# kharchenkolab/dropEst

Hardware: AMD Instinct MI355X
Metric: Mreads/s processed to final count matrix (higher is better)
Workload: dtype u64

## Files before the change

dropest_amd/capi.py:

```python
import ctypes as C
import os

import numpy as np

from .build import LIB, build

ESCAPE = 1 << 63
NO_GENE = 0xFFFFFFFF

MERGE_NONE, MERGE_REAL_BARCODES, MERGE_SIMPLE, MERGE_POISSON_REAL, MERGE_POISSON_SIMPLE, MERGE_ALL = 0, 1, 2, 3, 4, 5
BARCODES_INDROP, BARCODES_CONST = 0, 1
UMI_MERGE_SIMPLE, UMI_MERGE_DIRECTIONAL = 0, 1

_STATUS = {1: "INVALID", 2: "RANGE", 3: "DEVICE", 4: "UNSUPPORTED", 5: "IO"}


class MatrixBytes(C.Structure):
    _fields_ = [("ncols", C.c_uint64), ("nnz", C.c_uint64), ("colptr", C.c_void_p), ("row_delta", C.c_void_p), ("value", C.c_void_p),
                ("n_row_listed", C.c_uint64), ("row_listed_pos", C.c_void_p), ("row_listed_row", C.c_void_p),
                ("n_value_listed", C.c_uint64), ("value_listed_pos", C.c_void_p), ("value_listed_value", C.c_void_p)]


class DropestError(RuntimeError):
    def __init__(self, status, msg):
# ... 158 lines not shown
        "dropest_sort_layout": (C.c_int, [vp, C.POINTER(C.c_uint32)]),
        "dropest_stream": (vp, [vp]),
        "dropest_host_register": (C.c_int, [C.c_int, vp, C.c_uint64, P(vp)]),
        "dropest_host_unregister": (C.c_int, [C.c_int, vp]),
        "dropest_ingest": (C.c_int, [vp]),
        "dropest_ingest_summary_get": (C.c_int, [vp, P(IngestSummary)]),
        "dropest_ingest_summary_set": (C.c_int, [vp, P(IngestSummary)]),
        "dropest_gene_chr_table": (C.c_int, [vp, P(vp), u64p]),
        "dropest_shard_merge_search": (C.c_int, [vp, C.c_uint64, vp, vp, vp, C.c_uint64, vp, vp, u64p]),
        "dropest_shard_merge_pairs": (C.c_int, [vp, vp, vp]),
        "dropest_shard_merge_export": (C.c_int, [vp, u64p, vp, vp, P(vp), vp]),
        "dropest_shard_merge_intersect": (C.c_int, [vp, C.c_uint64, vp, vp, vp, vp, vp]),
        "dropest_shard_merge_decide": (C.c_int, [vp, vp, vp]),
        "dropest_merge_apply": (C.c_int, [C.c_uint64, C.c_uint64, vp, vp, vp, vp, vp, vp]),
        "dropest_shard_merge_finish": (C.c_int, [vp, C.c_uint64, vp, vp, vp, vp, vp, C.c_uint64, vp, vp, C.c_uint64, vp, vp, vp]),
        "dropest_synth_generate_host": (C.c_int, [P(SynthParams), C.c_uint64, C.c_uint64, vp, vp, vp, vp]),
        "dropest_synth_generate_device": (C.c_int, [P(SynthParams), C.c_int, C.c_uint64, C.c_uint64, vp, vp, vp, vp]),
        "dropest_dev_alloc": (C.c_int, [C.c_int, C.c_uint64, P(vp)]),
        "dropest_dev_free": (C.c_int, [C.c_int, vp]),
        "dropest_dev_copy_to_host": (C.c_int, [C.c_int, vp, vp, C.c_uint64]),
        "dropest_dev_copy_from_host": (C.c_int, [C.c_int, vp, vp, C.c_uint64]),
        "dropest_dev_count": (C.c_int, []),
        "dropest_dev_sync": (C.c_int, [C.c_int]),
        "dropest_rand_sequence": (C.c_int, [C.c_uint32, C.c_uint64, vp]),
        "dropest_table_sizes": (C.c_int, [vp, vp]),
        "dropest_shard_unique_id": (C.c_int, [vp]),
        "dropest_shard_create": (C.c_int, [P(Cfg), C.c_int32, C.c_int32, vp, P(vp)]),
        "dropest_shard_group_create": (C.c_int, [P(Cfg), C.c_int32, vp, vp]),
        "dropest_shard_destroy": (None, [vp]),
        "dropest_shard_ctx": (vp, [vp]),
        "dropest_shard_set_reads_device": (C.c_int, [vp, vp, vp, vp, vp, C.c_uint64, C.c_uint64]),
        "dropest_shard_step": (C.c_int, [vp]),
        "dropest_shard_push_reads": (C.c_int, [vp, vp, vp, vp, vp, C.c_uint64, C.c_uint64]),
        "dropest_shard_push_reads_device": (C.c_int, [vp, vp, vp, vp, vp, C.c_uint64, C.c_uint64, C.c_int32, vp]),
        "dropest_deal_range": (C.c_int, [C.c_uint64, C.c_uint64, C.c_uint64, C.c_int32, vp, P(C.c_uint32)]),
        "dropest_reserve_reads": (C.c_int, [vp, C.c_uint64]),
        "dropest_shard_group_step": (C.c_int, [vp, C.c_int32]),
        "dropest_shard_merge_validation_samples": (C.c_int, [vp, P(ValidationOpts), P(ValidationSample), C.c_uint32]),
        "dropest_shard_group_merge_validation_samples": (C.c_int, [vp, C.c_int32, P(ValidationOpts), P(ValidationSample), C.c_uint32]),
        "dropest_validation_cut_pairs": (C.c_int, [vp, C.c_uint64, C.c_int32, vp]),
        "dropest_shard_read_corrections": (C.c_int, [vp, u64p, u64p, P(vp), P(vp), P(vp)]),
        "dropest_shard_group_read_corrections": (C.c_int, [vp, C.c_int32]),
        "dropest_shard_group_read_corrections_host": (C.c_int, [vp, C.c_int32, C.c_uint64, C.c_uint64, vp, vp, vp]),
        "dropest_shard_group_read_correction_counts": (C.c_int, [vp, C.c_int32, vp]),
        "dropest_shard_filtered_barcodes_device": (C.c_int, [vp, u64p, P(vp)]),
        "dropest_shard_matrix": (C.c_int, [vp, C.c_int, u64p, u64p, P(vp), P(vp), P(vp), P(vp)]),
# ... 15 lines not shown
    return L


EXPORTED_SYMBOLS = [
    "dropest_last_error", "dropest_cfg_defaults", "dropest_ctx_create", "dropest_ctx_destroy",
    "dropest_set_side_strings", "dropest_push_reads", "dropest_push_reads_device", "dropest_set_initialized",
    "dropest_merge_and_filter", "dropest_reset_results", "dropest_total_cells", "dropest_real_cells",
    "dropest_cell_rows", "dropest_cell_id_by_cb", "dropest_filtered_cells", "dropest_merge_targets",
    "dropest_global_counters", "dropest_cell_molecules", "dropest_molecules", "dropest_count_matrix",
    "dropest_count_matrix_csc", "dropest_count_matrix_csc_levels", "dropest_owner_of", "dropest_partition_by_owner", "dropest_partition_scratch_bytes", "dropest_clear_reads",
    "dropest_count_matrix_device", "dropest_cell_first_reads_device", "dropest_assemble_columns", "dropest_assemble_columns_async",
    "dropest_real_candidate_rows", "dropest_dev_copy_device", "dropest_umi_distribution",
    "dropest_collisions_adjusted_sizes", "dropest_poisson_intersection_prob", "dropest_poisson_upper_tail",
    "dropest_merge_validation", "dropest_merge_validation_samples",
    "dropest_shard_merge_validation_samples", "dropest_shard_group_merge_validation_samples", "dropest_validation_cut_pairs",
    "dropest_set_umi_qualities", "dropest_umi_quality_length", "dropest_cell_molecule_qualities",
    "dropest_set_umi_qualities_var", "dropest_cell_molecule_quality_lengths",
    "dropest_exclude_cell", "dropest_merge_cells", "dropest_merge_umis",
    "dropest_chr_stats", "dropest_merge_target", "dropest_simple_merge_pairs", "dropest_kernel_stats", "dropest_set_profiling", "dropest_set_profiling_filter", "dropest_prefetch_raw_matrix", "dropest_radix_plan", "dropest_stream",
    "dropest_sort_layout", "dropest_host_register", "dropest_host_unregister", "dropest_ingest", "dropest_ingest_summary_get", "dropest_ingest_summary_set",
    "dropest_gene_chr_table", "dropest_shard_merge_search", "dropest_shard_merge_pairs", "dropest_shard_merge_export",
    "dropest_shard_merge_intersect", "dropest_shard_merge_decide", "dropest_merge_apply", "dropest_shard_merge_finish",
    "dropest_synth_generate_host", "dropest_synth_generate_device", "dropest_dev_alloc", "dropest_dev_free",
    "dropest_dev_copy_to_host", "dropest_dev_copy_from_host", "dropest_dev_count", "dropest_dev_sync",
    "dropest_rand_sequence", "dropest_table_sizes",
    "dropest_shard_unique_id", "dropest_shard_create", "dropest_shard_group_create", "dropest_shard_destroy", "dropest_shard_ctx",
    "dropest_shard_set_reads_device", "dropest_shard_push_reads", "dropest_shard_push_reads_device", "dropest_deal_range", "dropest_reserve_reads", "dropest_shard_step", "dropest_shard_group_step", "dropest_shard_matrix", "dropest_shard_matrix_form",
    "dropest_shard_merged_barcodes", "dropest_shard_phase_stats", "dropest_shard_set_option", "dropest_test_transport", "dropest_plan_columns",
    "dropest_key_width", "dropest_ctx_split", "dropest_shard_matrix_narrow", "dropest_shard_matrix_bytes", "dropest_add_umi_to_cell", "dropest_umi_first_seen", "dropest_resident_reads", "dropest_prefetch_raw_matrix_narrow", "dropest_narrow_matrix_possible", "dropest_count_matrix_csc_narrow",
    "dropest_prefetch_raw_matrix_bytes", "dropest_count_matrix_csc_bytes", "dropest_matrix_bytes_widen", "dropest_matrix_rider_widen", "dropest_set_raw_matrix_prefetch", "dropest_set_matrix_wire", "dropest_set_umi_dictionary", "dropest_debug_refresh", "dropest_push_reads_gather", "dropest_shard_set_umi_qualities", "dropest_shard_set_umi_qualities_var",
    "dropest_debug_poison_scratch", "dropest_debug_trim_pool", "dropest_debug_alloc_ordinal", "dropest_debug_alloc_site",
    "dropest_set_save_umi_merge_targets", "dropest_umi_merge_targets", "dropest_read_corrections", "dropest_read_corrections_host",
    "dropest_read_correction_counts", "dropest_cell_barcodes_device",
    "dropest_shard_read_corrections", "dropest_shard_group_read_corrections", "dropest_shard_group_read_corrections_host",
    "dropest_shard_group_read_correction_counts", "dropest_shard_filtered_barcodes_device",
]


_B2C = {"A": 0, "C": 1, "G": 2, "T": 3}


def pack_seq(s):
    if not s or len(s) > 31:
        return None
    c = 1
    for ch in s:
        b = _B2C.get(ch)
# ... 656 lines not shown
```

dropest_amd/csrc/dropest_amd.hip:

```cpp

#include "context.h"
extern "C" void dropest_bgzf_warm_up(void *stream);
#include "k_keyscatter.h"
#include "k_umidict.h"

#include <atomic>
#include <functional>
#include <map>
#include <mutex>

using namespace dropest;

static thread_local std::string g_last_error;

template <class F>
static dropest_status guarded(F &&f) {
	try {
		f();
		return DROPEST_OK;
	} catch (const InvalidError &e) { g_last_error = e.what(); return DROPEST_ERR_INVALID;
	} catch (const RangeError &e) { g_last_error = e.what(); return DROPEST_ERR_RANGE;
	} catch (const UnsupportedError &e) { g_last_error = e.what(); return DROPEST_ERR_UNSUPPORTED;
	} catch (const IoError &e) { g_last_error = e.what(); return DROPEST_ERR_IO;
	} catch (const DeviceError &e) { g_last_error = e.what(); return DROPEST_ERR_DEVICE;
// ... 878 lines not shown
	const u32 rounds = 256;
	std::vector<u32> h(size_t(rounds) * 64), got(size_t(rounds) * 64);
	u32 x = 2463534242u;
	for (u32 r = 0; r < rounds; ++r) {
		const u32 nd = 1u + r % 64u;
		for (u32 l = 0; l < 64; ++l) { x ^= x << 13; x ^= x >> 17; x ^= x << 5; h[size_t(r) * 64 + l] = (x >> 8) % nd; }
	}
	DevBuf<u32> d_in, d_out;
	d_in.alloc(h.size()); d_out.alloc(h.size());
	HIP_CHECK(hipMemcpyAsync(d_in.p, h.data(), h.size() * 4, hipMemcpyHostToDevice, stream));
	hipLaunchKernelGGL(ss_lds_order_probe_kernel, dim3(1), dim3(64), 0, stream, d_in.p, rounds, d_out.p);
	HIP_CHECK(hipGetLastError());
	HIP_CHECK(hipMemcpyAsync(got.data(), d_out.p, got.size() * 4, hipMemcpyDeviceToHost, stream));
	HIP_CHECK(stream_wait(stream));
	bool ordered = true;
	for (u32 r = 0; r < rounds && ordered; ++r) {
		u32 seen[64] = {0};
		for (u32 l = 0; l < 64; ++l) { const u32 d = h[size_t(r) * 64 + l]; if (got[size_t(r) * 64 + l] != seen[d]) ordered = false; ++seen[d]; }
	}
	if (!ordered) fprintf(stderr, "[dropest_amd] device %d: LDS atomics of one instruction are not applied in lane order here; the finishing sort of the splitter sort ranks with ballots (slower, same results)\n", device);
	return known[device] = ordered;
}

bool dropest_ctx::splitter_sort_reduce() {
	const u32 n = u32(n_reads);
	const SsPlan plan = ss_plan(n_reads, chr_from_gene, layout.val_bytes);
	if (!plan.applicable) return false;
	const int tb = plan.tb, fb1 = plan.fb1, fb2 = plan.fb2;
	const bool wide = fb2 > 9;
	const u32 F1 = 1u << fb1, Ff = 1u << fb2, F2 = F1 * Ff;
	const int ms = layout.mark_shift, VB = layout.val_bytes;
	(void)tb;
	uint64_t os_max = plan.os;
	if (const char *e = getenv("DROPEST_SSORT_OS")) os_max = uint64_t(std::max(1, atoi(e)));
	const u32 os = u32(std::max<uint64_t>(1, std::min<uint64_t>(os_max, uint64_t(n) / (uint64_t(F2) * 2))));
	const u32 n_sample = F2 * os;
	const u64 order_mask = ~((1ull << ms) - 1ull);
	const u64 varying = (counters.key_or ^ counters.key_and) & order_mask;
	const bool reserve = plan.reserve && !ss_no_reserve && keys_a.n >= plan.span && keys_b.n >= plan.span &&
	                     (!VB || (vals_a.bytes() >= plan.span && vals_b.bytes() >= plan.span));
	const size_t span = reserve ? size_t(plan.span) : size_t(n);

	HostStage hs(this, "splitter_sort");
	u64 *keys = keys_a.p, *keys_alt = keys_b.p;
	uint8_t *vals = reinterpret_cast<uint8_t *>(vals_a.p), *vals_alt = reinterpret_cast<uint8_t *>(vals_b.p);

	const bool in_l1 = keys_in_l1 && reserve;
	if (keys_in_l1 && !reserve) throw InvalidError("internal: keys partitioned by the key pass, but the sort does not place by reservation");
	const bool rebase = VB == 1 && ms == 0 && reserve && !in_l1 && !getenv("DROPEST_SS_NO_REBASE");
	const int VB2 = rebase ? 0 : VB, ms2 = rebase ? 3 : ms;
	const u64 rebase_mask = rebase ? ~((1ull << layout.umi_bits) - 1ull) : 0ull;
	if (!in_l1) {
		ss_sample_a.ensure(n_sample); ss_sample_b.ensure(n_sample); ss_fine.ensure(F2); ss_coarse.ensure(F1);
		timed("ss_sample", double(n_sample) * 16, [&] {
			hipLaunchKernelGGL(ss_sample_kernel, dim3(div_up(n_sample, 256)), dim3(256), 0, stream, keys, n, ms, n_sample, ss_sample_a.p);
		});
		ss_splitters_from_sample(n_sample, os, Ff, F2, varying >> ms);
	}

	const u32 n_tiles = div_up(n, SS_TILE);
	u32 nblocks = std::min<u32>(n_tiles, 1024);
	const u32 tpb = div_up(n_tiles, nblocks);
	nblocks = div_up(n_tiles, tpb);
	const u32 parts = std::max<u32>(1, std::min<u32>(16, 2048 / F1));
	ss_bucket_base.ensure(F2); ss_bucket_cnt.ensure(F2); scalars.ensure(16);
	HIP_CHECK(hipMemsetAsync(scalars.p, 0, 16, stream));
	u32 max_cnt = 0;
	static const u32 SMALL_MAX = [] { const char *e = getenv("DROPEST_SS_SMALL_MAX"); return e && atoi(e) >= 256 && atoi(e) <= 2048 ? u32(atoi(e)) : 2048u; }();
	const bool atomic_rank = lds_atomics_lane_ordered(cfg.device, stream);
	ss_tmp.ensure(span * 2 + 2); ss_n_loc.ensure(F2); ss_prefix.ensure(F2); ss_chunk.ensure(1024);
	SsLocalArgs a{};
	a.keys = keys; a.vals = vals; a.bucket_base = ss_bucket_base.p; a.bucket_cnt = ss_bucket_cnt.p; a.n_buckets = F2; a.ms = ms2;
	if (rebase) { a.rebase_coarse = ss_coarse.p; a.rebase_mask = rebase_mask; a.rebase_div = Ff; }
	a.t_key = keys_alt; a.t_reads = ss_tmp.p; a.t_agg = ss_tmp.p + span; a.n_loc = ss_n_loc.p;
	if (const char *e = getenv("DROPEST_SS_DEBUG")) a.debug = u32(atoi(e));
	a.order_flag = scalars.p + 2;
	a.atomic_below = u32(ms2 + layout.umi_bits);
	if (const char *e = getenv("DROPEST_SS_ATOMIC_BELOW")) a.atomic_below = u32(atoi(e));
	a.cap = SMALL_MAX; a.skip_above = SMALL_MAX;
	const bool fused_cg_off = getenv("DROPEST_SS_NO_FUSED_CG") != nullptr;
	const bool fuse_cg = !fused_cg_off;
	cg_from_sort = false;
	if (fuse_cg) {
		ss_cg_loc.ensure(F2); ss_cg_cnt.ensure(F2); ss_cg_prefix.ensure(F2);
		HIP_CHECK(hipMemsetAsync(ss_cg_loc.p, 0, size_t(F2) * 4, stream));
		a.cg_loc = ss_cg_loc.p; a.cg_shift = ms2 + layout.umi_bits;
	}
	auto launch_small = [&] {
		static const int wave_mode = [] { const char *e = getenv("DROPEST_SS_LOCAL_WAVE"); return e ? atoi(e) : 0; }();
		if ((wave_mode == 64 || wave_mode == 128) && atomic_rank) {
			const size_t lds1 = ss_local_lds_bytes(a.cap, wave_mode);
			timed(VB2 ? "ss_local:key+1B" : "ss_local:keys", double(n) * (8 + VB2), [&] {
				if (wave_mode == 64) { if (VB2) hipLaunchKernelGGL((ss_local_wave_kernel<64, 1, true>), dim3(F2), dim3(64), lds1, stream, a); else hipLaunchKernelGGL((ss_local_wave_kernel<64, 0, true>), dim3(F2), dim3(64), lds1, stream, a); }
				else { if (VB2) hipLaunchKernelGGL((ss_local_wave_kernel<128, 1, true>), dim3(F2), dim3(128), lds1, stream, a); else hipLaunchKernelGGL((ss_local_wave_kernel<128, 0, true>), dim3(F2), dim3(128), lds1, stream, a); }
			});
			return;
		}
		const size_t lds = ss_local_lds_bytes(a.cap, 256);
		timed(VB2 ? "ss_local:key+1B" : "ss_local:keys", double(n) * (8 + VB2), [&] {
			if (atomic_rank) { if (VB2) hipLaunchKernelGGL((ss_local_kernel<1, true>), dim3(F2), dim3(256), lds, stream, a); else hipLaunchKernelGGL((ss_local_kernel<0, true>), dim3(F2), dim3(256), lds, stream, a); }
			else if (VB2) hipLaunchKernelGGL(ss_local_kernel<1>, dim3(F2), dim3(256), lds, stream, a);
			else hipLaunchKernelGGL(ss_local_kernel<0>, dim3(F2), dim3(256), lds, stream, a);
		});
	};
	if (reserve) {
		const u32 cap1 = u32(plan.cap1), cap2 = u32(plan.cap2), CS1 = 32;
		ss_cursors.ensure(size_t(F1) * CS1 + F2);
		if (!in_l1) HIP_CHECK(hipMemsetAsync(ss_cursors.p, 0, (size_t(F1) * CS1 + F2) * 4, stream));
		else HIP_CHECK(hipMemcpyAsync(scalars.p + 3, ks_flag.p, 4, hipMemcpyDeviceToDevice, stream));
		u32 *cur1 = ss_cursors.p, *cur2 = ss_cursors.p + size_t(F1) * CS1;
		const u32 probe = [] { const char *e = getenv("DROPEST_SS_PROBE"); return e ? u32(atoi(e)) : 0u; }();
		const bool no256 = getenv("DROPEST_SS_NO_F256") != nullptr;
		const u32 rebase_bits = [] { const char *e = getenv("DROPEST_SS_REBASE_BITS"); return e ? u32(std::min(61, std::max(1, atoi(e)))) : 61u; }();
		const SsReserve r1{cur1, CS1, cap1, 0u, scalars.p + 3, probe, rebase_bits}, r2{cur2, 1u, cap2, 0u, scalars.p + 3, probe, 61u};
		if (!in_l1) timed(VB ? "ss_scatter:L1:key+1B" : "ss_scatter:L1:keys", double(n) * (8 + VB + 8 + VB2), [&] {
			auto go = [&](auto kernel) { hipLaunchKernelGGL(kernel, dim3(nblocks), dim3(SS_T), 0, stream, keys, vals, keys_alt, vals_alt, n, ms, fb1, ss_coarse.p, tpb, r1, rebase_mask); };
			if (rebase) { if (wide) go(ss_scatter_res_l1_kernel<1, 1024, true>); else if (fb1 <= 8 && !no256) go(ss_scatter_res_l1_kernel<1, 256, true>); else go(ss_scatter_res_l1_kernel<1, 512, true>); }
			else if (wide) { if (VB) go(ss_scatter_res_l1_kernel<1, 1024>); else go(ss_scatter_res_l1_kernel<0, 1024>); }
			else if (fb1 <= 8 && !no256) { if (VB) go(ss_scatter_res_l1_kernel<1, 256>); else go(ss_scatter_res_l1_kernel<0, 256>); }
			else { if (VB) go(ss_scatter_res_l1_kernel<1, 512>); else go(ss_scatter_res_l1_kernel<0, 512>); }
		});
		timed(VB2 ? "ss_scatter:L2:key+1B" : "ss_scatter:L2:keys", double(n) * 2 * (8 + VB2), [&] {
			auto go = [&](auto kernel) { hipLaunchKernelGGL(kernel, dim3(F1 * parts), dim3(SS_T), 0, stream, keys_alt, vals_alt, keys, vals, ms2, fb2, ss_fine.p, cur1, CS1, cap1, parts, r2,
			                                                 rebase ? ss_coarse.p : static_cast<const u64 *>(nullptr), rebase_mask); };
			if (wide) { if (VB2) go(ss_scatter_res_l2_kernel<1, 1024>); else go(ss_scatter_res_l2_kernel<0, 1024>); }
			else if (fb2 <= 8 && !no256) { if (VB2) go(ss_scatter_res_l2_kernel<1, 256>); else go(ss_scatter_res_l2_kernel<0, 256>); }
			else { if (VB2) go(ss_scatter_res_l2_kernel<1, 512>); else go(ss_scatter_res_l2_kernel<0, 512>); }
		});
		timed("ss_scan", double(F2) * 12, [&] {
			hipLaunchKernelGGL(ss_res_buckets_kernel, dim3(div_up(F2, 256)), dim3(256), 0, stream, cur2, F2, cap2, ss_bucket_base.p, ss_bucket_cnt.p, scalars.p);
		});
		launch_small();
		u32 head[4] = {0, 0, 0, 0};
		fetch(head, scalars.p, 16);
		max_cnt = head[0];
		if (head[3]) {
			stats["count:ss_reserve_overflow"].launches += 1;
			ss_no_reserve = true;
			build_keys(false);
			return splitter_sort_reduce();
		}
		if (max_cnt > SS_LOCAL_MAX) { build_keys(false, false); return false; }
	} else {
	rs_hist.ensure(size_t(F1) * nblocks); rs_row_total.ensure(1024); ss_base1.ensure(F1 + 1);
	timed("ss_hist:L1", double(n) * 8, [&] {
		if (wide) hipLaunchKernelGGL(ss_hist_l1_kernel<1024>, dim3(nblocks), dim3(SS_T), 0, stream, keys, n, ms, fb1, ss_coarse.p, tpb, rs_hist.p);
		else hipLaunchKernelGGL(ss_hist_l1_kernel<512>, dim3(nblocks), dim3(SS_T), 0, stream, keys, n, ms, fb1, ss_coarse.p, tpb, rs_hist.p);
	});
	timed("ss_scan", double(F1) * nblocks * 8, [&] {
		hipLaunchKernelGGL(rs_scan_rows_kernel, dim3(F1), dim3(256), 0, stream, rs_hist.p, nblocks, rs_row_total.p);
		if (wide) hipLaunchKernelGGL(ss_scan_totals_kernel<1024>, dim3(1), dim3(1024), 0, stream, rs_row_total.p, F1, n, ss_base1.p);
		else hipLaunchKernelGGL(ss_scan_totals_kernel<512>, dim3(1), dim3(512), 0, stream, rs_row_total.p, F1, n, ss_base1.p);
	});
	timed(VB ? "ss_scatter:L1:key+1B" : "ss_scatter:L1:keys", double(n) * 2 * (8 + VB), [&] {
		auto go = [&](auto kernel) { hipLaunchKernelGGL(kernel, dim3(nblocks), dim3(SS_T), 0, stream, keys, vals, keys_alt, vals_alt, n, ms, fb1, ss_coarse.p, tpb, rs_hist.p, ss_base1.p); };
		if (wide) { if (VB) go(ss_scatter_l1_kernel<1, 1024>); else go(ss_scatter_l1_kernel<0, 1024>); }
		else { if (VB) go(ss_scatter_l1_kernel<1, 512>); else go(ss_scatter_l1_kernel<0, 512>); }
	});

	ss_cnt2.ensure(size_t(F2) * parts);
	timed("ss_hist:L2", double(n) * 8, [&] {
		if (wide) hipLaunchKernelGGL(ss_hist_l2_kernel<1024>, dim3(F1 * parts), dim3(SS_T), 0, stream, keys_alt, ms, fb2, ss_fine.p, ss_base1.p, parts, ss_cnt2.p);
		else hipLaunchKernelGGL(ss_hist_l2_kernel<512>, dim3(F1 * parts), dim3(SS_T), 0, stream, keys_alt, ms, fb2, ss_fine.p, ss_base1.p, parts, ss_cnt2.p);
	});
	timed("ss_scan", double(F2) * parts * 8, [&] {
		if (wide) hipLaunchKernelGGL(ss_scan_seg_kernel<1024>, dim3(F1), dim3(1024), 0, stream, ss_cnt2.p, Ff, parts, ss_base1.p, ss_bucket_base.p, ss_bucket_cnt.p, scalars.p);
		else hipLaunchKernelGGL(ss_scan_seg_kernel<512>, dim3(F1), dim3(512), 0, stream, ss_cnt2.p, Ff, parts, ss_base1.p, ss_bucket_base.p, ss_bucket_cnt.p, scalars.p);
	});
	fetch(&max_cnt, scalars.p, 4);
	if (max_cnt > SS_LOCAL_MAX) return false;
	timed(VB ? "ss_scatter:L2:key+1B" : "ss_scatter:L2:keys", double(n) * 2 * (8 + VB), [&] {
		auto go = [&](auto kernel) { hipLaunchKernelGGL(kernel, dim3(F1 * parts), dim3(SS_T), 0, stream, keys_alt, vals_alt, keys, vals, ms, fb2, ss_fine.p, ss_base1.p, parts, ss_cnt2.p); };
		if (wide) { if (VB) go(ss_scatter_l2_kernel<1, 1024>); else go(ss_scatter_l2_kernel<0, 1024>); }
		else { if (VB) go(ss_scatter_l2_kernel<1, 512>); else go(ss_scatter_l2_kernel<0, 512>); }
	});
	}

	if (!reserve) launch_small();
	if (max_cnt > SMALL_MAX) {
		std::vector<u32> cnts(F2), medium, big;
		fetch(cnts.data(), ss_bucket_cnt.p, size_t(F2) * 4);
		for (u32 b = 0; b < F2; ++b) if (cnts[b] > SMALL_MAX) (cnts[b] <= 4096 ? medium : big).push_back(b);
		ss_big_list.ensure(medium.size() + big.size());
		if (!medium.empty()) HIP_CHECK(hipMemcpyAsync(ss_big_list.p, medium.data(), medium.size() * 4, hipMemcpyHostToDevice, stream));
		if (!big.empty()) HIP_CHECK(hipMemcpyAsync(ss_big_list.p + medium.size(), big.data(), big.size() * 4, hipMemcpyHostToDevice, stream));
		auto launch = [&](auto kernel, u32 threads, u32 cap, const u32 *list, size_t count) {
			SsLocalArgs g = a;
			g.big_list = list; g.cap = cap; g.skip_above = cap;
			const size_t lds = ss_local_lds_bytes(cap, int(threads));
			HIP_CHECK(hipFuncSetAttribute(reinterpret_cast<const void *>(kernel), hipFuncAttributeMaxDynamicSharedMemorySize, int(lds)));
			hipLaunchKernelGGL(kernel, dim3(u32(count)), dim3(threads), lds, stream, g);
		};
		timed("ss_local:big", 0, [&] {
			if (atomic_rank) {
				if (!medium.empty()) { if (VB2) launch(ss_local_big_kernel<256, 1, true>, 256, 4096, ss_big_list.p, medium.size()); else launch(ss_local_big_kernel<256, 0, true>, 256, 4096, ss_big_list.p, medium.size()); }
				if (!big.empty()) { if (VB2) launch(ss_local_big_kernel<512, 1, true>, 512, SS_LOCAL_MAX, ss_big_list.p + medium.size(), big.size()); else launch(ss_local_big_kernel<512, 0, true>, 512, SS_LOCAL_MAX, ss_big_list.p + medium.size(), big.size()); }
			} else {
				if (!medium.empty()) { if (VB2) launch(ss_local_big_kernel<256, 1>, 256, 4096, ss_big_list.p, medium.size()); else launch(ss_local_big_kernel<256, 0>, 256, 4096, ss_big_list.p, medium.size()); }
				if (!big.empty()) { if (VB2) launch(ss_local_big_kernel<512, 1>, 512, SS_LOCAL_MAX, ss_big_list.p + medium.size(), big.size()); else launch(ss_local_big_kernel<512, 0>, 512, SS_LOCAL_MAX, ss_big_list.p + medium.size(), big.size()); }
			}
		});
		HIP_CHECK(stream_wait(stream));
	}
	const u32 n_chunks = div_up(F2, 1024);
	timed("ss_scan", double(F2) * 12, [&] {
		hipLaunchKernelGGL(ss_chunk_sums_kernel<1024>, dim3(n_chunks), dim3(1024), 0, stream, ss_n_loc.p, F2, ss_chunk.p);
		hipLaunchKernelGGL(ss_prefix_kernel<1024>, dim3(n_chunks), dim3(1024), 0, stream, ss_n_loc.p, F2, ss_chunk.p, n_chunks, ss_prefix.p, scalars.p + 1);
		if (fuse_cg) {
			hipLaunchKernelGGL(ss_cg_counts_kernel, dim3(div_up(F2, 256)), dim3(256), 0, stream, ss_bucket_base.p, ss_n_loc.p, keys_alt, layout.umi_bits, F2, ss_cg_loc.p, ss_cg_cnt.p);
			hipLaunchKernelGGL(ss_chunk_sums_kernel<1024>, dim3(n_chunks), dim3(1024), 0, stream, ss_cg_cnt.p, F2, ss_chunk.p);
			hipLaunchKernelGGL(ss_prefix_kernel<1024>, dim3(n_chunks), dim3(1024), 0, stream, ss_cg_cnt.p, F2, ss_chunk.p, n_chunks, ss_cg_prefix.p, scalars.p + 4);
		}
// ... 1780 lines not shown
```

dropest_amd/csrc/k_ssort.h:

```cpp
#pragma once

#include "util.h"

namespace dropest {

constexpr int SS_T = 512, SS_I = 8, SS_TILE = SS_T * SS_I;
constexpr int SS_MAX_F = 512;
constexpr uint32_t SS_LOCAL_MAX = 8192;

__global__ __launch_bounds__(256) void ss_sample_kernel(const unsigned long long *__restrict__ keys, uint32_t n, int ms,
                                                        uint32_t n_sample, unsigned long long *__restrict__ out) {
	const uint32_t j = blockIdx.x * 256 + threadIdx.x;
	if (j >= n_sample) return;
	const uint32_t pos = uint32_t((uint64_t(j) * n + n / 2) / n_sample);
	out[j] = keys[pos < n ? pos : n - 1] >> ms;
}

__global__ __launch_bounds__(256) void ss_pick_splitters_kernel(const unsigned long long *__restrict__ sorted_sample, uint32_t os, uint32_t F, uint32_t F2,
                                                                unsigned long long *__restrict__ fine, unsigned long long *__restrict__ coarse) {
	const uint32_t j = blockIdx.x * 256 + threadIdx.x;
	if (j >= F2) return;
	const unsigned long long v = j + 1 < F2 ? sorted_sample[size_t(j + 1) * os] : ~0ull;
	fine[j] = v;
	if ((j + 1) % F == 0) coarse[(j + 1) / F - 1] = v;
// ... 294 lines not shown
			if (g < (rs.first + d + 1u) * rs.cap) {
				if constexpr (REBASE) {
					const unsigned long long diff = sk[q] - (d ? (sp[d - 1u] & rebase_mask) : 0ull);
					if (diff >> rs.rebase_bits) atomicOr(rs.overflow, 1u);
					okeys[g] = (diff << 3) | (unsigned long long)(sv[q] & 7u);
				} else {
					okeys[g] = sk[q];
					if (VB) ovals[g] = sv[q];
				}
			}
		}
		if ((rs.dbg & 2u) && t0 + SS_TILE < end) load_tile(t0 + SS_TILE);
		lds_barrier();
	}
}

#define SS_SCATTER_RES_LDS(VB, MAXF)                                                                        \
	__shared__ unsigned long long sp[MAXF];                                                                 \
	__shared__ uint32_t cnt[MAXF], tstart[MAXF], gdelta[MAXF], scratch[SS_T / 64 + 1];                      \
	__shared__ unsigned long long sk[SS_TILE];                                                              \
	__shared__ uint16_t sd[SS_TILE];                                                                        \
	__shared__ uint8_t sv[VB ? SS_TILE : 1];

template <int VB, int MAXF, bool REBASE = false>
__global__ __launch_bounds__(SS_T) void ss_scatter_res_l1_kernel(const unsigned long long *__restrict__ keys, const uint8_t *__restrict__ vals,
                                                                 unsigned long long *__restrict__ okeys, uint8_t *__restrict__ ovals, uint32_t n,
                                                                 int ms, int fb, const unsigned long long *__restrict__ coarse,
                                                                 uint32_t tiles_per_block, SsReserve rs, unsigned long long rebase_mask) {
	SS_SCATTER_RES_LDS(VB, MAXF)
	const uint32_t F = 1u << fb;
	for (uint32_t j = threadIdx.x; j < F; j += SS_T) sp[j] = j + 1 < F ? coarse[j] : ~0ull;
	__syncthreads();
	const uint64_t b64 = uint64_t(blockIdx.x) * tiles_per_block * SS_TILE;
	uint64_t e64 = b64 + uint64_t(tiles_per_block) * SS_TILE;
	if (e64 > n) e64 = n;
	if (b64 < n) ss_scatter_res_range<VB, MAXF, REBASE>(keys, vals, okeys, ovals, uint32_t(b64), uint32_t(e64), ms, fb, sp, rs, cnt, tstart, gdelta, scratch, sk, sd, sv, rebase_mask);
}
template <int VB, int MAXF>
__global__ __launch_bounds__(SS_T) void ss_scatter_res_l2_kernel(const unsigned long long *__restrict__ keys, const uint8_t *__restrict__ vals,
                                                                 unsigned long long *__restrict__ okeys, uint8_t *__restrict__ ovals, int ms, int fb,
                                                                 const unsigned long long *__restrict__ fine, const uint32_t *__restrict__ cur1,
                                                                 uint32_t cstride1, uint32_t cap1, uint32_t parts, SsReserve rs,
                                                                 const unsigned long long *__restrict__ rebase_coarse, unsigned long long rebase_mask) {
	SS_SCATTER_RES_LDS(VB, MAXF)
	const uint32_t F = 1u << fb, s = blockIdx.x / parts, p = blockIdx.x % parts;
	const unsigned long long lo = (rebase_coarse && s) ? (rebase_coarse[s - 1] & rebase_mask) : 0ull;
	for (uint32_t j = threadIdx.x; j < F; j += SS_T) {
		const unsigned long long f = j + 1 < F ? fine[size_t(s) * F + j] : ~0ull;
		sp[j] = j + 1 < F ? (f > lo ? f - lo : 0ull) : ~0ull;
	}
	__syncthreads();
	const uint32_t fill = cur1[size_t(s) * cstride1], sb = s * cap1, se = sb + (fill < cap1 ? fill : cap1);
	const uint32_t tiles = (se - sb + SS_TILE - 1) / SS_TILE, tpp = (tiles + parts - 1) / parts;
	const uint64_t b = uint64_t(sb) + uint64_t(p) * tpp * SS_TILE, e = b + uint64_t(tpp) * SS_TILE;
	const uint32_t begin = b < se ? uint32_t(b) : se, end = e < se ? uint32_t(e) : se;
	SsReserve mine = rs;
	mine.first = s * F;
	if (begin < end) ss_scatter_res_range<VB, MAXF>(keys, vals, okeys, ovals, begin, end, ms, fb, sp, mine, cnt, tstart, gdelta, scratch, sk, sd, sv);
}
__global__ __launch_bounds__(256) void ss_res_buckets_kernel(const uint32_t *__restrict__ cur2, uint32_t n_buckets, uint32_t cap,
                                                             uint32_t *__restrict__ bucket_base, uint32_t *__restrict__ bucket_cnt, uint32_t *__restrict__ max_cnt) {
	const uint32_t b = blockIdx.x * 256 + threadIdx.x;
// ... 17 lines not shown
	uint32_t *order_flag;
	unsigned long long *t_key;
	uint32_t *t_reads, *t_agg, *n_loc;
	uint32_t *cg_loc;
	int cg_shift;
	const unsigned long long *rebase_coarse;
	unsigned long long rebase_mask;
	uint32_t rebase_div;
};

template <int THREADS, int ITEMS, int VB, bool ATOMIC_RANK = false>
__device__ inline void ss_local_run(const SsLocalArgs &a, uint32_t bucket, uint32_t base, uint32_t cnt, unsigned char *smem) {
	constexpr uint32_t WAVES = THREADS / 64;
	const uint32_t tid = threadIdx.x, w = tid >> 6, lane = tid & 63u;
	unsigned long long *sk = reinterpret_cast<unsigned long long *>(smem);
	uint32_t *agg = reinterpret_cast<uint32_t *>(smem);
	uint32_t *headpos = agg + a.cap;
	uint32_t *wcnt = reinterpret_cast<uint32_t *>(smem + size_t(a.cap) * 8);
	uint32_t *tstart = wcnt + WAVES * 256;
	uint32_t *scratch = tstart + 256;
	uint32_t *wtot = scratch + (THREADS / 64 + 1);
	uint32_t *misc = wtot + WAVES;
	unsigned long long *red = reinterpret_cast<unsigned long long *>(misc + 4 + ((WAVES + 1) & 1u));
	uint8_t *sv = reinterpret_cast<uint8_t *>(red + 2 * WAVES);
	const int ms = a.ms;
	const uint32_t coarse_b = a.rebase_coarse ? bucket / a.rebase_div : 0u;
	const unsigned long long kbase = coarse_b ? (a.rebase_coarse[coarse_b - 1u] & a.rebase_mask) : 0ull;

	const uint32_t lane_off = w * (64 * ITEMS) + lane;
	unsigned long long key[ITEMS];
	uint8_t val[VB ? ITEMS : 1];
	unsigned long long k_or = 0, k_and = ~0ull;
#pragma unroll
	for (int i = 0; i < ITEMS; ++i) {
		const uint32_t p = lane_off + i * 64;
		const bool valid = p < cnt;
		key[i] = valid ? a.keys[base + p] : 0ull;
		if (VB) val[i] = valid ? a.vals[base + p] : uint8_t(0);
	}
#pragma unroll
	for (int i = 0; i < ITEMS; ++i) {
		const uint32_t p = lane_off + i * 64;
		if (p < cnt) { k_or |= key[i]; k_and &= key[i]; sk[p] = key[i]; if (VB) sv[p] = val[i]; }
	}
	k_or = wave_reduce_or_u64(k_or); k_and = wave_reduce_and_u64(k_and);
	if (lane == 0) { red[2 * w] = k_or; red[2 * w + 1] = k_and; }
	lds_barrier();
// ... 107 lines not shown
		const uint32_t m = woff + pre[i] + is_head - 1u;
		const uint32_t mark = VB ? uint32_t(val[i]) & 7u : uint32_t(key[i]) & 7u;
		if (is_head) { headpos[m] = p; a.t_key[base + m] = (key[i] >> ms) + kbase; }
		const uint32_t add = (((mark >> 1) & 1u) << 1) | (((mark >> 2) & 1u) << 16);
		if (add) atomicAdd(&agg[m], add);
		if (mark & 1u) atomicOr(&agg[m], 1u);
	}
	lds_barrier();
	for (uint32_t m = tid; m < n_loc; m += THREADS) {
		const uint32_t e = m + 1 < n_loc ? headpos[m + 1] : cnt;
		a.t_reads[base + m] = e - headpos[m];
		a.t_agg[base + m] = agg[m];
	}
}

template <int VB, bool ATOMIC_RANK = false>
__global__ __launch_bounds__(256) void ss_local_kernel(SsLocalArgs a) {
	extern __shared__ __attribute__((aligned(16))) unsigned char ss_smem[];
	const uint32_t b = blockIdx.x;
	const uint32_t cnt = a.bucket_cnt[b], base = a.bucket_base[b];
	if (cnt == 0) { if (threadIdx.x == 0) a.n_loc[b] = 0; return; }
	if (cnt > a.skip_above) return;
	if (cnt <= 1024) ss_local_run<256, 4, VB, ATOMIC_RANK>(a, b, base, cnt, ss_smem);
	else ss_local_run<256, 8, VB, ATOMIC_RANK>(a, b, base, cnt, ss_smem);
}
template <int THREADS, int VB, bool ATOMIC_RANK = false>
__global__ __launch_bounds__(THREADS) void ss_local_wave_kernel(SsLocalArgs a) {
	extern __shared__ __attribute__((aligned(16))) unsigned char ss_smem[];
	const uint32_t b = blockIdx.x;
	const uint32_t cnt = a.bucket_cnt[b], base = a.bucket_base[b];
	if (cnt == 0) { if (threadIdx.x == 0) a.n_loc[b] = 0; return; }
	if (cnt > a.skip_above) return;
	if (cnt <= 1024) ss_local_run<THREADS, 1024 / THREADS, VB, ATOMIC_RANK>(a, b, base, cnt, ss_smem);
	else ss_local_run<THREADS, 2048 / THREADS, VB, ATOMIC_RANK>(a, b, base, cnt, ss_smem);
}
template <int THREADS, int VB, bool ATOMIC_RANK = false>
__global__ __launch_bounds__(THREADS) void ss_local_big_kernel(SsLocalArgs a) {
	extern __shared__ __attribute__((aligned(16))) unsigned char ss_smem[];
	const uint32_t b = a.big_list[blockIdx.x];
	ss_local_run<THREADS, 16, VB, ATOMIC_RANK>(a, b, a.bucket_base[b], a.bucket_cnt[b], ss_smem);
}

inline size_t ss_local_lds_bytes(uint32_t cap, int threads) {
	const size_t waves = size_t(threads) / 64;
	size_t words = waves * 256 + 256 + (size_t(threads) / 64 + 1) + waves + 4 + ((waves + 1) & 1u);
	return size_t(cap) * 8 + words * 4 + 2 * waves * 8 + size_t(cap) + 16;
}

__global__ __launch_bounds__(64) void ss_lds_order_probe_kernel(const uint32_t *__restrict__ digit, uint32_t rounds, uint32_t *__restrict__ out) {
	__shared__ uint32_t cnt[64];
	for (uint32_t r = 0; r < rounds; ++r) {
		cnt[threadIdx.x] = 0;
		__builtin_amdgcn_wave_barrier();
		out[r * 64 + threadIdx.x] = atomicAdd(&cnt[digit[r * 64 + threadIdx.x] & 63u], 1u);
		__builtin_amdgcn_wave_barrier();
	}
}

template <int MAXF>
__global__ __launch_bounds__(MAXF) void ss_chunk_sums_kernel(const uint32_t *__restrict__ n_loc, uint32_t n_buckets, uint32_t *__restrict__ chunk_sum) {
	__shared__ uint32_t scratch[MAXF / 64 + 1];
	const uint32_t i = blockIdx.x * MAXF + threadIdx.x;
	uint32_t total;
	block_excl_scan_u32<MAXF>(i < n_buckets ? n_loc[i] : 0u, scratch, total);
	if (threadIdx.x == 0) chunk_sum[blockIdx.x] = total;
}
template <int MAXF>
__global__ __launch_bounds__(MAXF) void ss_prefix_kernel(const uint32_t *__restrict__ n_loc, uint32_t n_buckets, const uint32_t *__restrict__ chunk_sum,
                                                          uint32_t n_chunks, uint32_t *__restrict__ prefix, uint32_t *__restrict__ n_mol) {
// ... 225 lines not shown
```

dropest_amd/csrc/synth_api.hip:

```cpp

#include "synth.h"

#include <cstring>

using namespace dropest;

extern "C" {

int dropest_synth_generate_host(const dropest_synth_params *p, uint64_t first, uint64_t n, uint64_t *cb, uint64_t *umi,
                                uint32_t *gene, uint32_t *aux) {
	if (!p || !p->cell_cb || !p->cell_cdf || !p->gene_cdf || p->n_cells == 0 || p->n_genes == 0 || p->n_chr == 0 ||
	    p->cb_len == 0 || p->cb_len > 31 || p->umi_len == 0 || p->umi_len > 31 || p->reads_per_molecule == 0)
		return 1;
	for (uint64_t i = 0; i < n; ++i) {
		const SynthRead r = synth_read(*p, p->cell_cb, p->cell_cdf, p->gene_cdf, first + i);
		cb[i] = r.cb; umi[i] = r.umi; gene[i] = r.gene; aux[i] = r.aux;
	}
	return 0;
}

int dropest_synth_generate_device(const dropest_synth_params *p, int device, uint64_t first, uint64_t n, uint64_t *d_cb,
                                  uint64_t *d_umi, uint32_t *d_gene, uint32_t *d_aux) {
	if (!p || !p->cell_cb || !p->cell_cdf || !p->gene_cdf || p->n_cells == 0 || p->n_genes == 0 || p->n_chr == 0 ||
	    p->cb_len == 0 || p->cb_len > 31 || p->umi_len == 0 || p->umi_len > 31 || p->reads_per_molecule == 0)
// ... 5 lines not shown
		HIP_CHECK(hipMemcpy(ccb.p, p->cell_cb, size_t(p->n_cells) * 8, hipMemcpyHostToDevice));
		HIP_CHECK(hipMemcpy(ccdf.p, p->cell_cdf, size_t(p->n_cells) * 4, hipMemcpyHostToDevice));
		HIP_CHECK(hipMemcpy(gcdf.p, p->gene_cdf, size_t(p->n_genes) * 4, hipMemcpyHostToDevice));
		if (n) {
			const uint64_t want = (n + 255) / 256;
			const unsigned blocks = unsigned(want < 8192 ? want : 8192);
			hipLaunchKernelGGL(synth_kernel, dim3(blocks), dim3(256), 0, nullptr, *p, ccb.p, ccdf.p, gcdf.p, first, n, d_cb,
			                   d_umi, d_gene, d_aux);
			HIP_CHECK(hipGetLastError());
		}
		HIP_CHECK(hipDeviceSynchronize());
		return 0;
	} catch (const std::exception &e) {
		std::fprintf(stderr, "dropest_synth_generate_device: %s\n", e.what());
		return 2;
	}
}

int dropest_dev_count(void) {
	int n = 0;
	if (hipGetDeviceCount(&n) != hipSuccess) return 0;
	return n;
}
int dropest_dev_alloc(int device, uint64_t bytes, void **out) {
	if (hipSetDevice(device) != hipSuccess) return 1;
	return hipMalloc(out, bytes ? bytes : 1) == hipSuccess ? 0 : 2;
}
int dropest_dev_free(int device, void *p) {
	if (hipSetDevice(device) != hipSuccess) return 1;
	return hipFree(p) == hipSuccess ? 0 : 2;
}
int dropest_dev_copy_to_host(int device, void *dst, const void *d_src, uint64_t bytes) {
	if (hipSetDevice(device) != hipSuccess) return 1;
	return hipMemcpy(dst, d_src, bytes, hipMemcpyDeviceToHost) == hipSuccess ? 0 : 2;
}
int dropest_dev_copy_from_host(int device, void *d_dst, const void *src, uint64_t bytes) {
	if (hipSetDevice(device) != hipSuccess) return 1;
	return hipMemcpy(d_dst, src, bytes, hipMemcpyHostToDevice) == hipSuccess ? 0 : 2;
}
int dropest_dev_sync(int device) {
	if (hipSetDevice(device) != hipSuccess) return 1;
	return hipDeviceSynchronize() == hipSuccess ? 0 : 2;
}

}
```

include/dropest_synth.h:

```cpp
#ifndef DROPEST_SYNTH_H
#define DROPEST_SYNTH_H

#include <stdint.h>

#ifdef __cplusplus
extern "C" {
#endif

typedef struct {
	uint64_t seed;
	uint32_t stream_id;
	uint32_t n_cells;
	const uint64_t *cell_cb;
	const uint32_t *cell_cdf;
	uint32_t n_genes;
	const uint32_t *gene_cdf;
	uint32_t cb_len, umi_len;
	uint32_t n_chr;
	uint32_t permille_neighbour, permille_ambient, permille_intergenic;
	uint32_t permille_intron, permille_exon_na;
	uint64_t n_effective;
	uint32_t reads_per_molecule;
} dropest_synth_params;

int dropest_synth_generate_host(const dropest_synth_params *p, uint64_t first, uint64_t n, uint64_t *cb,
                                uint64_t *umi, uint32_t *gene, uint32_t *aux);
int dropest_synth_generate_device(const dropest_synth_params *p, int device, uint64_t first, uint64_t n,
                                  uint64_t *d_cb, uint64_t *d_umi, uint32_t *d_gene, uint32_t *d_aux);

int dropest_dev_alloc(int device, uint64_t bytes, void **out);
int dropest_dev_free(int device, void *p);
int dropest_dev_copy_to_host(int device, void *dst, const void *d_src, uint64_t bytes);
int dropest_dev_copy_from_host(int device, void *d_dst, const void *src, uint64_t bytes);
int dropest_dev_count(void);
int dropest_dev_sync(int device);

#ifdef __cplusplus
}
#endif
#endif
```

Measured before the change: 11530.

## Raise splitter-sort occupancy via LDS trimming, launch bounds, and mid-size local tier

The local sort kernels no longer reserve LDS for value bytes when there are no values, which lowers per-workgroup LDS and can allow more resident workgroups per CU. The reserve scatter kernels gain a minimum-waves launch bound (6 for key-only with fan-out up to 512) that caps register use to raise occupancy, at some risk of spills. A new 6-items-per-thread tier handles buckets of 1025-1536 keys, avoiding the 8-item path there. Profiling hooks that query occupancy and an LDS-per-CU device query are also added.

```diff
diff --git a/dropest_amd/capi.py b/dropest_amd/capi.py
--- a/dropest_amd/capi.py
+++ b/dropest_amd/capi.py
@@ -204,6 +204,7 @@
         "dropest_dev_copy_from_host": (C.c_int, [C.c_int, vp, vp, C.c_uint64]),
         "dropest_dev_count": (C.c_int, []),
         "dropest_dev_sync": (C.c_int, [C.c_int]),
+        "dropest_dev_lds_per_cu": (C.c_uint64, [C.c_int]),
         "dropest_rand_sequence": (C.c_int, [C.c_uint32, C.c_uint64, vp]),
         "dropest_table_sizes": (C.c_int, [vp, vp]),
         "dropest_shard_unique_id": (C.c_int, [vp]),
@@ -265,7 +266,7 @@
     "dropest_gene_chr_table", "dropest_shard_merge_search", "dropest_shard_merge_pairs", "dropest_shard_merge_export",
     "dropest_shard_merge_intersect", "dropest_shard_merge_decide", "dropest_merge_apply", "dropest_shard_merge_finish",
     "dropest_synth_generate_host", "dropest_synth_generate_device", "dropest_dev_alloc", "dropest_dev_free",
-    "dropest_dev_copy_to_host", "dropest_dev_copy_from_host", "dropest_dev_count", "dropest_dev_sync",
+    "dropest_dev_copy_to_host", "dropest_dev_copy_from_host", "dropest_dev_count", "dropest_dev_sync", "dropest_dev_lds_per_cu",
     "dropest_rand_sequence", "dropest_table_sizes",
     "dropest_shard_unique_id", "dropest_shard_create", "dropest_shard_group_create", "dropest_shard_destroy", "dropest_shard_ctx",
     "dropest_shard_set_reads_device", "dropest_shard_push_reads", "dropest_shard_push_reads_device", "dropest_deal_range", "dropest_reserve_reads", "dropest_shard_step", "dropest_shard_group_step", "dropest_shard_matrix", "dropest_shard_matrix_form",
diff --git a/dropest_amd/csrc/dropest_amd.hip b/dropest_amd/csrc/dropest_amd.hip
--- a/dropest_amd/csrc/dropest_amd.hip
+++ b/dropest_amd/csrc/dropest_amd.hip
@@ -924,6 +924,17 @@
 	return known[device] = ordered;
 }
 
+static u32 ss_workgroups_per_cu(const void *kernel, int threads, size_t lds) {
+	static std::mutex mu;
+	static std::map<std::pair<const void *, size_t>, u32> known;
+	std::lock_guard<std::mutex> lk(mu);
+	auto it = known.find({kernel, lds});
+	if (it != known.end()) return it->second;
+	int per_cu = 0;
+	HIP_CHECK(hipOccupancyMaxActiveBlocksPerMultiprocessor(&per_cu, kernel, threads, lds));
+	return known[{kernel, lds}] = u32(std::max(0, per_cu));
+}
+
 bool dropest_ctx::splitter_sort_reduce() {
 	const u32 n = u32(n_reads);
 	const SsPlan plan = ss_plan(n_reads, chr_from_gene, layout.val_bytes);
@@ -964,6 +975,20 @@
 	u32 nblocks = std::min<u32>(n_tiles, 1024);
 	const u32 tpb = div_up(n_tiles, nblocks);
 	nblocks = div_up(n_tiles, tpb);
+	const bool no256 = getenv("DROPEST_SS_NO_F256") != nullptr;
+	auto with_res_l2_kernel = [&](auto &&f) {
+		if (wide) { if (VB2) f(ss_scatter_res_l2_kernel<1, 1024>); else f(ss_scatter_res_l2_kernel<0, 1024>); }
+		else if (fb2 <= 8 && !no256) { if (VB2) f(ss_scatter_res_l2_kernel<1, 256>); else f(ss_scatter_res_l2_kernel<0, 256>); }
+		else { if (VB2) f(ss_scatter_res_l2_kernel<1, 512>); else f(ss_scatter_res_l2_kernel<0, 512>); }
+	};
+	auto with_cnt_l2_kernel = [&](auto &&f) {
+		if (wide) { if (VB) f(ss_scatter_l2_kernel<1, 1024>); else f(ss_scatter_l2_kernel<0, 1024>); }
+		else { if (VB) f(ss_scatter_l2_kernel<1, 512>); else f(ss_scatter_l2_kernel<0, 512>); }
+	};
+	if (profiling) {
+		auto ask = [&](auto kernel) { stats["count:ss_l2_workgroups_per_cu"].launches = ss_workgroups_per_cu(reinterpret_cast<const void *>(kernel), SS_T, 0); };
+		if (reserve) with_res_l2_kernel(ask); else with_cnt_l2_kernel(ask);
+	}
 	const u32 parts = std::max<u32>(1, std::min<u32>(16, 2048 / F1));
 	ss_bucket_base.ensure(F2); ss_bucket_cnt.ensure(F2); scalars.ensure(16);
 	HIP_CHECK(hipMemsetAsync(scalars.p, 0, 16, stream));
@@ -991,18 +1016,22 @@
 	auto launch_small = [&] {
 		static const int wave_mode = [] { const char *e = getenv("DROPEST_SS_LOCAL_WAVE"); return e ? atoi(e) : 0; }();
 		if ((wave_mode == 64 || wave_mode == 128) && atomic_rank) {
-			const size_t lds1 = ss_local_lds_bytes(a.cap, wave_mode);
+			const size_t lds1 = ss_local_lds_bytes(a.cap, wave_mode, VB2);
 			timed(VB2 ? "ss_local:key+1B" : "ss_local:keys", double(n) * (8 + VB2), [&] {
 				if (wave_mode == 64) { if (VB2) hipLaunchKernelGGL((ss_local_wave_kernel<64, 1, true>), dim3(F2), dim3(64), lds1, stream, a); else hipLaunchKernelGGL((ss_local_wave_kernel<64, 0, true>), dim3(F2), dim3(64), lds1, stream, a); }
 				else { if (VB2) hipLaunchKernelGGL((ss_local_wave_kernel<128, 1, true>), dim3(F2), dim3(128), lds1, stream, a); else hipLaunchKernelGGL((ss_local_wave_kernel<128, 0, true>), dim3(F2), dim3(128), lds1, stream, a); }
 			});
 			return;
 		}
-		const size_t lds = ss_local_lds_bytes(a.cap, 256);
+		const size_t lds = ss_local_lds_bytes(a.cap, 256, VB2);
+		auto with_kernel = [&](auto &&f) {
+			if (atomic_rank) { if (VB2) f(ss_local_kernel<1, true>); else f(ss_local_kernel<0, true>); }
+			else if (VB2) f(ss_local_kernel<1>);
+			else f(ss_local_kernel<0>);
+		};
+		if (profiling) with_kernel([&](auto kernel) { stats["count:ss_local_workgroups_per_cu"].launches = ss_workgroups_per_cu(reinterpret_cast<const void *>(kernel), 256, lds); });
 		timed(VB2 ? "ss_local:key+1B" : "ss_local:keys", double(n) * (8 + VB2), [&] {
-			if (atomic_rank) { if (VB2) hipLaunchKernelGGL((ss_local_kernel<1, true>), dim3(F2), dim3(256), lds, stream, a); else hipLaunchKernelGGL((ss_local_kernel<0, true>), dim3(F2), dim3(256), lds, stream, a); }
-			else if (VB2) hipLaunchKernelGGL(ss_local_kernel<1>, dim3(F2), dim3(256), lds, stream, a);
-			else hipLaunchKernelGGL(ss_local_kernel<0>, dim3(F2), dim3(256), lds, stream, a);
+			with_kernel([&](auto kernel) { hipLaunchKernelGGL(kernel, dim3(F2), dim3(256), lds, stream, a); });
 		});
 	};
 	if (reserve) {
@@ -1012,7 +1041,6 @@
 		else HIP_CHECK(hipMemcpyAsync(scalars.p + 3, ks_flag.p, 4, hipMemcpyDeviceToDevice, stream));
 		u32 *cur1 = ss_cursors.p, *cur2 = ss_cursors.p + size_t(F1) * CS1;
 		const u32 probe = [] { const char *e = getenv("DROPEST_SS_PROBE"); return e ? u32(atoi(e)) : 0u; }();
-		const bool no256 = getenv("DROPEST_SS_NO_F256") != nullptr;
 		const u32 rebase_bits = [] { const char *e = getenv("DROPEST_SS_REBASE_BITS"); return e ? u32(std::min(61, std::max(1, atoi(e)))) : 61u; }();
 		const SsReserve r1{cur1, CS1, cap1, 0u, scalars.p + 3, probe, rebase_bits}, r2{cur2, 1u, cap2, 0u, scalars.p + 3, probe, 61u};
 		if (!in_l1) timed(VB ? "ss_scatter:L1:key+1B" : "ss_scatter:L1:keys", double(n) * (8 + VB + 8 + VB2), [&] {
@@ -1025,9 +1053,7 @@
 		timed(VB2 ? "ss_scatter:L2:key+1B" : "ss_scatter:L2:keys", double(n) * 2 * (8 + VB2), [&] {
 			auto go = [&](auto kernel) { hipLaunchKernelGGL(kernel, dim3(F1 * parts), dim3(SS_T), 0, stream, keys_alt, vals_alt, keys, vals, ms2, fb2, ss_fine.p, cur1, CS1, cap1, parts, r2,
 			                                                 rebase ? ss_coarse.p : static_cast<const u64 *>(nullptr), rebase_mask); };
-			if (wide) { if (VB2) go(ss_scatter_res_l2_kernel<1, 1024>); else go(ss_scatter_res_l2_kernel<0, 1024>); }
-			else if (fb2 <= 8 && !no256) { if (VB2) go(ss_scatter_res_l2_kernel<1, 256>); else go(ss_scatter_res_l2_kernel<0, 256>); }
-			else { if (VB2) go(ss_scatter_res_l2_kernel<1, 512>); else go(ss_scatter_res_l2_kernel<0, 512>); }
+			with_res_l2_kernel(go);
 		});
 		timed("ss_scan", double(F2) * 12, [&] {
 			hipLaunchKernelGGL(ss_res_buckets_kernel, dim3(div_up(F2, 256)), dim3(256), 0, stream, cur2, F2, cap2, ss_bucket_base.p, ss_bucket_cnt.p, scalars.p);
@@ -1073,8 +1099,7 @@
 	if (max_cnt > SS_LOCAL_MAX) return false;
 	timed(VB ? "ss_scatter:L2:key+1B" : "ss_scatter:L2:keys", double(n) * 2 * (8 + VB), [&] {
 		auto go = [&](auto kernel) { hipLaunchKernelGGL(kernel, dim3(F1 * parts), dim3(SS_T), 0, stream, keys_alt, vals_alt, keys, vals, ms, fb2, ss_fine.p, ss_base1.p, parts, ss_cnt2.p); };
-		if (wide) { if (VB) go(ss_scatter_l2_kernel<1, 1024>); else go(ss_scatter_l2_kernel<0, 1024>); }
-		else { if (VB) go(ss_scatter_l2_kernel<1, 512>); else go(ss_scatter_l2_kernel<0, 512>); }
+		with_cnt_l2_kernel(go);
 	});
 	}
 
@@ -1089,7 +1114,7 @@
 		auto launch = [&](auto kernel, u32 threads, u32 cap, const u32 *list, size_t count) {
 			SsLocalArgs g = a;
 			g.big_list = list; g.cap = cap; g.skip_above = cap;
-			const size_t lds = ss_local_lds_bytes(cap, int(threads));
+			const size_t lds = ss_local_lds_bytes(cap, int(threads), VB2);
 			HIP_CHECK(hipFuncSetAttribute(reinterpret_cast<const void *>(kernel), hipFuncAttributeMaxDynamicSharedMemorySize, int(lds)));
 			hipLaunchKernelGGL(kernel, dim3(u32(count)), dim3(threads), lds, stream, g);
 		};
diff --git a/dropest_amd/csrc/k_ssort.h b/dropest_amd/csrc/k_ssort.h
--- a/dropest_amd/csrc/k_ssort.h
+++ b/dropest_amd/csrc/k_ssort.h
@@ -340,8 +340,9 @@
 	__shared__ uint16_t sd[SS_TILE];                                                                        \
 	__shared__ uint8_t sv[VB ? SS_TILE : 1];
 
+#define SS_RES_MIN_WAVES(VB, MAXF) ((VB) == 0 && (MAXF) <= 512 ? 6 : 2)
 template <int VB, int MAXF, bool REBASE = false>
-__global__ __launch_bounds__(SS_T) void ss_scatter_res_l1_kernel(const unsigned long long *__restrict__ keys, const uint8_t *__restrict__ vals,
+__global__ __launch_bounds__(SS_T, SS_RES_MIN_WAVES(VB, MAXF)) void ss_scatter_res_l1_kernel(const unsigned long long *__restrict__ keys, const uint8_t *__restrict__ vals,
                                                                  unsigned long long *__restrict__ okeys, uint8_t *__restrict__ ovals, uint32_t n,
                                                                  int ms, int fb, const unsigned long long *__restrict__ coarse,
                                                                  uint32_t tiles_per_block, SsReserve rs, unsigned long long rebase_mask) {
@@ -355,7 +356,7 @@
 	if (b64 < n) ss_scatter_res_range<VB, MAXF, REBASE>(keys, vals, okeys, ovals, uint32_t(b64), uint32_t(e64), ms, fb, sp, rs, cnt, tstart, gdelta, scratch, sk, sd, sv, rebase_mask);
 }
 template <int VB, int MAXF>
-__global__ __launch_bounds__(SS_T) void ss_scatter_res_l2_kernel(const unsigned long long *__restrict__ keys, const uint8_t *__restrict__ vals,
+__global__ __launch_bounds__(SS_T, SS_RES_MIN_WAVES(VB, MAXF)) void ss_scatter_res_l2_kernel(const unsigned long long *__restrict__ keys, const uint8_t *__restrict__ vals,
                                                                  unsigned long long *__restrict__ okeys, uint8_t *__restrict__ ovals, int ms, int fb,
                                                                  const unsigned long long *__restrict__ fine, const uint32_t *__restrict__ cur1,
                                                                  uint32_t cstride1, uint32_t cap1, uint32_t parts, SsReserve rs,
@@ -419,7 +420,7 @@
 	uint32_t *wtot = scratch + (THREADS / 64 + 1);
 	uint32_t *misc = wtot + WAVES;
 	unsigned long long *red = reinterpret_cast<unsigned long long *>(misc + 4 + ((WAVES + 1) & 1u));
-	uint8_t *sv = reinterpret_cast<uint8_t *>(red + 2 * WAVES);
+	uint8_t *sv = VB ? reinterpret_cast<uint8_t *>(red + 2 * WAVES) : nullptr;
 	const int ms = a.ms;
 	const uint32_t coarse_b = a.rebase_coarse ? bucket / a.rebase_div : 0u;
 	const unsigned long long kbase = coarse_b ? (a.rebase_coarse[coarse_b - 1u] & a.rebase_mask) : 0ull;
@@ -573,6 +574,7 @@
 	if (cnt == 0) { if (threadIdx.x == 0) a.n_loc[b] = 0; return; }
 	if (cnt > a.skip_above) return;
 	if (cnt <= 1024) ss_local_run<256, 4, VB, ATOMIC_RANK>(a, b, base, cnt, ss_smem);
+	else if (cnt <= 1536) ss_local_run<256, 6, VB, ATOMIC_RANK>(a, b, base, cnt, ss_smem);
 	else ss_local_run<256, 8, VB, ATOMIC_RANK>(a, b, base, cnt, ss_smem);
 }
 template <int THREADS, int VB, bool ATOMIC_RANK = false>
@@ -592,10 +594,10 @@
 	ss_local_run<THREADS, 16, VB, ATOMIC_RANK>(a, b, a.bucket_base[b], a.bucket_cnt[b], ss_smem);
 }
 
-inline size_t ss_local_lds_bytes(uint32_t cap, int threads) {
+inline size_t ss_local_lds_bytes(uint32_t cap, int threads, int vb) {
 	const size_t waves = size_t(threads) / 64;
 	size_t words = waves * 256 + 256 + (size_t(threads) / 64 + 1) + waves + 4 + ((waves + 1) & 1u);
-	return size_t(cap) * 8 + words * 4 + 2 * waves * 8 + size_t(cap) + 16;
+	return size_t(cap) * 8 + words * 4 + 2 * waves * 8 + (vb ? size_t(cap) : 0) + 16;
 }
 
 __global__ __launch_bounds__(64) void ss_lds_order_probe_kernel(const uint32_t *__restrict__ digit, uint32_t rounds, uint32_t *__restrict__ out) {
diff --git a/dropest_amd/csrc/synth_api.hip b/dropest_amd/csrc/synth_api.hip
--- a/dropest_amd/csrc/synth_api.hip
+++ b/dropest_amd/csrc/synth_api.hip
@@ -51,6 +51,11 @@
 	if (hipGetDeviceCount(&n) != hipSuccess) return 0;
 	return n;
 }
+uint64_t dropest_dev_lds_per_cu(int device) {
+	int bytes = 0;
+	if (hipDeviceGetAttribute(&bytes, hipDeviceAttributeMaxSharedMemoryPerMultiprocessor, device) != hipSuccess || bytes < 0) return 0;
+	return uint64_t(bytes);
+}
 int dropest_dev_alloc(int device, uint64_t bytes, void **out) {
 	if (hipSetDevice(device) != hipSuccess) return 1;
 	return hipMalloc(out, bytes ? bytes : 1) == hipSuccess ? 0 : 2;
diff --git a/include/dropest_synth.h b/include/dropest_synth.h
--- a/include/dropest_synth.h
+++ b/include/dropest_synth.h
@@ -34,6 +34,7 @@
 int dropest_dev_copy_from_host(int device, void *d_dst, const void *src, uint64_t bytes);
 int dropest_dev_count(void);
 int dropest_dev_sync(int device);
+uint64_t dropest_dev_lds_per_cu(int device);
 
 #ifdef __cplusplus
 }
```

New measurement: 11510. No clear change (-0.2%).
